# facebookresearch/holo_diffusion

Measured on AMD Instinct MI355X. Metric: denoise-steps/sec + rendered-rays/sec, 64^3x32 grid @400^2 render, higher is better.
Workload: dtype f32

## Files before the change

### holo_diffusion_amd/csrc/holo_kernels.h

```cpp
#pragma once
#include <stddef.h>
#include <stdint.h>

#include "conv_weights.h"
#include "holo_knobs.h"

struct HoloCtx {
  int device;
  int num_cus;
  int deterministic = 0;
};

namespace holo {

enum class ConvKernel : int32_t {
  Gather = 0,
  Halo = 1,
  RowTile = 2,
  Wino2 = 4,
  Bf16Wide = 5,
  Wino3 = 6,
  Stream1x1 = 7,
  Bf16Persistent = 8,
  S2Bf16 = 9,
// ... 11 lines not shown
  int OD, OH, OW;
  int stride, pad, ksz;
  int Cout;
  const float* w;
  int CoutP, CinP;
  const float* coef;
  int act;
  const float* bias;
  const float* residual;
  float* out;
  const float* skip_src0;
  const float* skip_src1;
  int skip_C0, skip_C1;
  const float* skip_w;
  const uint16_t* w_bf;
  const uint16_t* skip_w_bf;
  int bf16;
  int skip_CinP;
  const float* skip_bias;
  double* stats;
  float* partial;
  int nsplit;
  int chunks_per_split;
  int skip_chunks_per_split;
  int tz;
  int grid_x;
  int stagger_ticks;
  unsigned long long* dbg;
  ConvKernel kernel;
  const float* w_wino2;
  const float* skip_w_wino2;
  const float* w_wino3;
  const float* skip_w_wino3;
  const uint16_t* w_bft;
  const uint16_t* skip_w_bft;
  int in_bf16;
  int res_bf16;
  int out_bf16;
  uint16_t* qkv_q;
  uint16_t* qkv_k;
  uint16_t* qkv_vt;
  float qkv_scale;
  int qkv_T, qkv_CH, qkv_H;
  int qkv_sb, qkv_rows;
};

bool conv_s2_bf16_supported(const ConvParams& p);
int conv_s2_bf16_launch(const ConvParams& p, void* stream);

bool conv1x1_qkv_bf16_supported(const ConvParams& p);
void conv1x1_qkv_bf16_plan(ConvParams& p, int num_cus);
int conv1x1_qkv_bf16_launch(const ConvParams& p, void* stream);
bool conv1x1_bf16_stream_supported(const ConvParams& p);
void conv1x1_bf16_stream_plan(ConvParams& p, int num_cus);
int conv1x1_bf16_stream_slabs(const ConvParams& p);
int conv1x1_bf16_stream_launch(const ConvParams& p, void* stream);

int repack_conv_weight_wino3_launch(const float* w, float* out, int Cout, int Cin, int src_taps, int CoutP, int CinP,
                                    void* stream);
int conv_wino3_launch(const ConvParams& p, void* stream);
int conv_bf16p_launch(const ConvParams& p, void* stream);

size_t conv_plan(ConvParams& p, int num_cus, const Knobs& k, int plan_n = 0);
int conv_launch(const ConvParams& p, void* stream);
int conv_stats_slabs(const ConvParams& p);
double conv_flops(const ConvParams& p);
// ... 375 lines not shown
```

### holo_diffusion_amd/csrc/holo_knobs.h

```cpp
#pragma once

#include <stdint.h>
#include <stdlib.h>

namespace holo {

#ifdef HOLO_EMU
constexpr bool EMU_BUILD = true;
#else
constexpr bool EMU_BUILD = false;
#endif

constexpr int64_t KNOB_UNSET = INT64_MIN;

#define HOLO_KNOBS(X)                                                                                                      \
  X(num_cus, "HOLO_NUM_CUS", POS, 0, CTX, "planners size grids and split-K for this many CUs (default: the device's)")     \
  X(conv_wino, "HOLO_CONV_WINO", INT, 1, HANDLE, "0: no Winograd copies of the conv weights (forward and dgrad)")          \
  X(conv_wino3, "HOLO_CONV_WINO3", INT, 1, HANDLE_PLAN, "0: no F(2x2x2, 3x3x3) copies / conv_wino3_kernel never chosen")   \
  X(keep_intermediates, "HOLO_KEEP_INTERMEDIATES", CH, '1', HANDLE,                                                        \
    "1: the plan releases no activation, holo_unet_fetch_block works")                                                     \
  X(render_v1, "HOLO_RENDER_V1", SET, 0, HANDLE, "the ray-per-column render kernel for everything")                        \
  X(render2_nw, "HOLO_RENDER2_NW", INT, 0, HANDLE, "8: the 8-wave form of render2_kernel's 12-wave configurations")        \
  X(render2_nrm_nw, "HOLO_RENDER2_NRM_NW", INT, 0, HANDLE,                                                                 \
    "8: rendered normals two waves per SIMD instead of 10 waves (the emulation build always runs 8)")                      \
  X(render_wgs, "HOLO_RENDER_WGS", POS, 0, HANDLE, "persistent render workgroups (default: one per CU)")                   \
  X(render_xcd, "HOLO_RENDER_XCD", RAW, KNOB_UNSET, HANDLE,                                                                \
    "XCD ranges of the render tile order (default 8; 2 in the emulation build; <= 1: plain order)")                        \
  X(render_tail, "HOLO_RENDER_TAIL", RAW, KNOB_UNSET, HANDLE,                                                              \
    "4-ray tiles at the end of every XCD range handed out as single rays (default: about two rounds; 3 in the "            \
    "emulation build; 0: off)")                                                                                            \
  X(render_static_tiles, "HOLO_RENDER_STATIC_TILES", SET, 0, HANDLE, "static tile stride instead of the dynamic hand-out") \
  X(render_timeline, "HOLO_RENDER_TIMELINE", SET, 0, HANDLE, "per-phase clocks of every render launch (synchronises!)")    \
  X(mlp_mean_bwd_chunk, "HOLO_MLP_MEAN_BWD_CHUNK", POS, 0, HANDLE,                                                         \
    "voxels per chunk of holo_mlp_mean_backward (default: what fits 4 GiB of rows; the emulation build: always 2048)")     \
  X(conv_wino_small, "HOLO_CONV_WINO_SMALL", INT, 1, PLAN, "0: under-filled levels take 64-voxel tiles, not Winograd")     \
  X(conv_force_tz2, "HOLO_CONV_FORCE_TZ2", INT, 0, PLAN, "1: 128-voxel tiles (hence the Winograd kernels) on small grids") \
  X(conv_qkv_fused, "HOLO_CONV_QKV_FUSED", INT, 1, PLAN, "0: row-tile qkv convolution + attn_pack_kernel")                 \
  X(conv1x1_bf16_stream, "HOLO_CONV1X1_BF16_STREAM", INT, 1, PLAN, "0: the row-tile kernel for bf16 1x1x1 convolutions")   \
  X(conv1x1_stream_min_m, "HOLO_CONV1X1_STREAM_MIN_M", INT, 131072, PLAN,                                                  \
    "rows from which a raw-input fp32 1x1x1 convolution streams (0: never)")                                               \
  X(conv1x1_small, "HOLO_CONV1X1_SMALL", INT, 1, PLAN, "0: the row-tile kernel for the fp32 attention's 1x1x1 convs")      \
  X(conv_s2t, "HOLO_CONV_S2T", INT, -1, PLAN, "stride-2 bf16 halo kernel: 0 never, 1 wherever defined (default: by fill)") \
  X(conv_bf16t, "HOLO_CONV_BF16T", INT, -1, PLAN, "bf16 wide-tile kernel: 0 never, 1 everywhere (default: by fill / K)")   \
  X(conv_bf16p, "HOLO_CONV_BF16P", INT, -1, PLAN,                                                                          \
    "its persistent form: 0 never, 1 every wide-tile launch, 2 activated input too (default: raw input)")                  \
  X(conv_bf16p_wgs, "HOLO_CONV_BF16P_WGS", INT, 0, PLAN, "at most this many persistent workgroups (0: no cap)")            \
  X(conv_wino3_min_items, "HOLO_CONV_WINO3_MIN_ITEMS", INT, KNOB_UNSET, PLAN,                                              \
    "work items from which conv_wino3_kernel runs (default: num_cus / 2)")                                                 \
  X(no_skip_fusion, "HOLO_NO_SKIP_FUSION", SET, 0, PLAN, "a ResBlock's 1x1x1 skip always as its own launch")               \
  X(skip_fusion_below_r, "HOLO_SKIP_FUSION_BELOW_R", RAW, 64, PLAN,                                                        \
    "exact fp32: the skip is fused into the second convolution below this grid edge")                                      \
  X(no_flash_attn, "HOLO_NO_FLASH_ATTN", SET, 0, PLAN, "attention as GEMM + softmax + GEMM")                               \
  X(bf16_flash_min_t, "HOLO_BF16_FLASH_MIN_T", RAW, 1024, PLAN, "tokens from which the bf16 mode takes its bf16 attention") \
  X(flash_split, "HOLO_FLASH_SPLIT", INT, 0, PLAN, "key splits of the fp32 attention, clamped to [1, T/128] (0: by fill)") \
  X(flash_v2_ksplit, "HOLO_FLASH_V2_KSPLIT", INT, 0, PLAN,                                                                 \
    "key splits of the bf16 attention: 1..8 dividing T into multiples of 128, else ignored")                               \
  X(attn_exact, "HOLO_ATTN_EXACT", SET, 0, PLAN, "bf16 attention: the exact loop alone, no LAZY pass")                     \
  X(debug_timestep_load, "HOLO_DEBUG_TIMESTEP_LOAD", INT, 0, PLAN, "how time_embed_kernel loads the timesteps (see it)")   \
  X(dgrad_s2_direct, "HOLO_DGRAD_S2_DIRECT", CH, '1', PLAN, "1: conv_dgrad_s2_kernel for every Downsample dgrad")          \
  X(wgrad_tiles, "HOLO_WGRAD_TILES", POS, 0, PLAN, "> 0: the tile weight-gradient kernel instead of the row-staged one")   \
  X(wgrad_reduce_tile_min, "HOLO_WGRAD_REDUCE_TILE_MIN", RAW, 1024, PLAN,                                                  \
    "64-element tiles from which the weight-gradient reduce runs its tile form")                                           \
  X(debug_plan, "HOLO_DEBUG_PLAN", SET, 0, PLAN, "[plan] lines on stderr: what every convolution / attention launches")    \
  X(viewpool_bwd_v1, "HOLO_VIEWPOOL_BWD_V1", CH, '1', CALL, "1: the register-accumulating view-pool backward kernel")      \
  HOLO_KNOBS_DEV(X)

#ifdef HOLO_DEV_PROBES
#define HOLO_KNOBS_DEV(X)                                                                                                  \
  X(viewpool_bwd_probe, "HOLO_VIEWPOOL_BWD_PROBE", RAW, KNOB_UNSET, CALL,                                                  \
    "view-pool backward: 0 no pass 2, 2 pass 2 without its atomics, 10 + k the atomics of map k alone")                    \
  X(viewpool_bwd_occ, "HOLO_VIEWPOOL_BWD_OCC", CH, '3', CALL, "view-pool backward: 3 = the 166-register build")
#else
#define HOLO_KNOBS_DEV(X)
#endif

typedef int64_t knob_INT_t, knob_RAW_t, knob_POS_t;
typedef bool knob_SET_t, knob_CH_t;
static inline int64_t knob_INT(const char* e, int64_t dflt) { return e && e[0] ? strtoll(e, nullptr, 10) : dflt; }
static inline int64_t knob_RAW(const char* e, int64_t dflt) { return e ? atoll(e) : dflt; }
static inline bool knob_SET(const char* e, int) { return e != nullptr; }
static inline bool knob_CH(const char* e, char c) { return e && e[0] == c; }
// ... 17 lines not shown
```

### holo_diffusion_amd/csrc/kernels_conv.hip

```cpp
#include <stdio.h>
#include <stdlib.h>

#include "holo_common.h"
#include "holo_kernels.h"

namespace holo {

namespace {

constexpr int BM = 128;
constexpr int BK = 32;
constexpr int LDK = 36;

__device__ __forceinline__ float silu_f(float v) { return v / (1.0f + __expf(-v)); }
__device__ __forceinline__ float silu_fast(float v) { return v * holo_rcp(1.0f + __expf(-v)); }

__device__ __forceinline__ float bf16_load(const uint16_t* p) { return __uint_as_float((uint32_t)(*p) << 16); }
__device__ __forceinline__ uint16_t bf16_round(float v) { return (uint16_t)(pack_bf16x2(v, 0.f) & 0xffffu); }
__device__ __forceinline__ float4 ld_act4(const float* base, int64_t idx, int bf) {
  if (bf) {
    const uint2 u = *reinterpret_cast<const uint2*>(reinterpret_cast<const uint16_t*>(base) + idx);
    return make_float4(__uint_as_float(u.x << 16), __uint_as_float(u.x & 0xffff0000u), __uint_as_float(u.y << 16),
                       __uint_as_float(u.y & 0xffff0000u));
  }
// ... 2326 lines not shown
      const int64_t s2t = k.conv_s2t;
      if (s2t != 0 && conv_s2_bf16_supported(p) && ((Mc / 128) * (p.Cout / 64) >= num_cus / 4 || s2t == 1))
        return ConvKernel::S2Bf16;
      return p.Cout >= 64 ? ConvKernel::RowTile : ConvKernel::Gather;
    }
    const int64_t bt = k.conv_bf16t;
    if (p.bf16 == 1 && p.in_bf16 && p.w_bft && (!p.skip_w || p.skip_w_bft) && (p.OD % 8) == 0 && (p.OH % 8) == 0 &&
        (p.OW % 8) == 0 && (p.Cout % 32) == 0 && (p.C0 % 8) == 0 && (p.skip_C0 % 8) == 0 && ((p.skip_C0 + p.skip_C1) % 8) == 0 &&
        (p.Cout >= 64 || !p.skip_w) && bt != 0 &&
        (t8 >= target || Cin + (p.skip_w ? p.skip_C0 + p.skip_C1 : 0) >= BF16T_LONG_K || bt == 1)) {
      const int64_t bp = k.conv_bf16p;
      const int wgs = num_cus & ~7;
      if (bp != 0 && (bp == 1 || bp == 2 || !p.coef) &&
          ((bf16t_split(p, t8, ncc16, num_cus).n == 1 && wgs >= 8 && t8 >= wgs) || bp == 1) &&
          (p.C1 == 0 || (p.C0 % 16) == 0) &&
          (!p.skip_w || (((p.skip_C0 + p.skip_C1) % 32) == 0 && (p.skip_C1 == 0 || (p.skip_C0 % 32) == 0))) &&
          src_vox < ((int64_t)1 << 24))
        return ConvKernel::Bf16Persistent;
      return ConvKernel::Bf16Wide;
    }
    if (tz == 2 && k.conv_wino3 != 0 && p.w_wino3 && p.bf16 == 0 && !p.in_bf16 && !p.out_bf16 && p.Cout >= 64 &&
        (p.Cout % 64) == 0 && (!p.skip_w || p.skip_w_wino3) && (p.OH % 8) == 0 && (p.OW % 8) == 0 && (p.OD % 2) == 0 &&
        (!p.coef || p.act) &&
        (int64_t)p.N * src_vox * (cmax > skmax ? cmax : skmax) * 4 < ((int64_t)1 << 32) &&
        (int64_t)wino3_split(t3, ncc, num_cus).n * Mc * p.Cout * 4 < ((int64_t)1 << 32) &&
        (!p.stats || (Mc / 128) * p.Cout * 16 < ((int64_t)1 << 32)) &&
        (!p.skip_w || ((p.skip_C0 % 16) == 0 && (p.skip_C1 % 4) == 0)) &&
        t3 * wino3_split(t3, ncc, num_cus).n >= (k.conv_wino3_min_items != KNOB_UNSET ? k.conv_wino3_min_items : num_cus / 2))
      return ConvKernel::Wino3;
    if (tz == 2 && (wino2_wide || (p.w_wino2 && p.bf16 == 0 && p.Cout == 32 && !p.skip_w))) return ConvKernel::Wino2;
    return ConvKernel::Halo;
  }();
  p.kernel = kernel;

  switch (kernel) {
    case ConvKernel::Qkv:
    case ConvKernel::Bf16Stream1x1:
    case ConvKernel::Stream1x1:
    case ConvKernel::Small1x1:
      p.nsplit = 1;
      p.chunks_per_split = ncc;
      if (kernel == ConvKernel::Qkv) conv1x1_qkv_bf16_plan(p, num_cus);
      if (kernel == ConvKernel::Bf16Stream1x1) conv1x1_bf16_stream_plan(p, num_cus);
      break;
    case ConvKernel::S2Bf16:
      p.nsplit = 1;
      p.chunks_per_split = Cin / 16;
      break;
    case ConvKernel::RowTile: {
      const int64_t t2 = cdiv(Mc, SM_ROWS) * cdiv(p.Cout, 64);
      const int64_t tgt = SM_SPLIT_WGS_PER_CU * (int64_t)num_cus;
      const int nall = nchunks + nsk;
      const int max_split = nall / SG > 1 ? nall / SG : 1;
      const KSplit s = ksplit(t2 < tgt ? cdiv(tgt, t2) : 1, max_split, nall);
      p.nsplit = s.n;
      p.chunks_per_split = s.cps;
      break;
    }
    case ConvKernel::Gather: {
      const int max_split = nchunks / 4 > 1 ? nchunks / 4 : 1;
      const KSplit s = ksplit(tiles < target ? cdiv(target, tiles) : 1, max_split, nchunks);
      p.nsplit = s.n;
      p.chunks_per_split = s.cps;
      break;
    }
    case ConvKernel::Bf16Wide: {
// ... 54 lines not shown
    int B, vpb;
    gn_stats_geometry(p.Cout < 1024 ? p.Cout : 1024, V, &B, &vpb);
    return B;
  }
  switch (p.kernel) {
    case ConvKernel::Bf16Wide:
    case ConvKernel::Bf16Persistent:
      return (int)(V / 512);
    case ConvKernel::Halo:
      if (p.bf16 == 2 && p.w_bf && p.Cout >= 64 && !p.skip_w) return (int)(V / 32);
      [[fallthrough]];
    case ConvKernel::Wino2:
    case ConvKernel::Wino3:
      return (int)(V / (64 * p.tz)) * (p.Cout >= 64 ? 1 : 2);
    case ConvKernel::RowTile:
      return V % SM_ROWS == 0 ? (int)(V / SM_ROWS) : 0;
    case ConvKernel::S2Bf16:
      return (int)(V / 128);
    case ConvKernel::Bf16Stream1x1:
      return conv1x1_bf16_stream_slabs(p);
    case ConvKernel::Small1x1:
      return (int)(V / 16);
    default:
      return 0;
  }
}

double conv_flops(const ConvParams& p) {
  const double M = (double)p.N * p.OD * p.OH * p.OW;
  return 2.0 * M * p.Cout * ((double)(p.C0 + p.C1) * p.ksz * p.ksz * p.ksz + (p.skip_w ? p.skip_C0 + p.skip_C1 : 0));
}

double conv_exec_flops(const ConvParams& p) {
  const double taps = p.kernel == ConvKernel::Wino3 ? 8.0 : p.kernel == ConvKernel::Wino2 ? 12.0 : 0.0;
  if (taps == 0.0) return conv_flops(p);
  const double M = (double)p.N * p.OD * p.OH * p.OW;
  return 2.0 * M * p.Cout * ((double)(p.C0 + p.C1) * taps + (p.skip_w ? p.skip_C0 + p.skip_C1 : 0));
}

int conv_launch(const ConvParams& p, void* stream) {
  const int Cin = p.C0 + p.C1;
  if ((Cin & 3) || (p.C0 & 3) || (p.Cout & 3) || (p.src1 && (p.C0 % BK))) {
    set_error("conv_launch: unsupported channel counts C0=%d C1=%d Cout=%d", p.C0, p.C1, p.Cout);
    return -1;
  }
  if (p.nsplit > 1 && !p.partial) {
    set_error("conv_launch: split-K without scratch");
    return -1;
  }
  const int64_t M = (int64_t)p.N * p.OD * p.OH * p.OW;
  const bool wide = p.Cout >= 64;
  const bool sk = p.skip_w != nullptr;
  const int bn = wide ? 64 : 32;
  dim3 block(256);
  dim3 hgrid((unsigned)p.grid_x, (unsigned)cdiv(p.Cout, bn), (unsigned)p.nsplit);
  switch (p.kernel) {
    case ConvKernel::Gather: {
      dim3 grid((unsigned)cdiv(M, BM), (unsigned)cdiv(p.Cout, bn), (unsigned)p.nsplit);
      if (wide) {
        HOLO_LAUNCH(conv_igemm_kernel<2>, grid, block, stream, p);
      } else {
        HOLO_LAUNCH(conv_igemm_kernel<1>, grid, block, stream, p);
      }
      break;
    }
    case ConvKernel::Halo: {
      if (p.bf16 == 2 && p.w_bf && wide && !sk) {
// ... 157 lines not shown
```

### holo_diffusion_amd/csrc/kernels_conv3.hip

```cpp
#include <stdio.h>
#include <stdlib.h>

#include <type_traits>
#include <utility>

#include "holo_common.h"
#include "holo_kernels.h"

#ifndef W3_PROBE
#define W3_PROBE 0
#endif
#ifndef W3_WDIST
#define W3_WDIST 3
#endif
#ifndef W3_ENTRY
#define W3_ENTRY conv_wino3_launch
#endif

namespace holo {

namespace {

#ifdef HOLO_EMU
#define W3_KARGS(kp) const ConvParams* kp = &p
#else
#define W3_KARGS(kp)                                                                                        \
  auto kp = (const ConvParams __attribute__((address_space(4)))*)(__builtin_amdgcn_kernarg_segment_ptr()); \
  asm volatile("" : "+s"(kp))
#endif

constexpr int W3_BK = 32;
constexpr int W3_RS = 36;
constexpr int W3_HY = 10, W3_HX = 10;
constexpr int W3_PLANE = W3_HY * W3_HX;
constexpr int W3_HALO = 4 * W3_PLANE * W3_RS;
constexpr int W3_WSUB = 4 * 256;
constexpr int W3_WCHUNK = 32 * W3_WSUB;
constexpr int W3_WSKIP = 4 * W3_WSUB;

__device__ __forceinline__ float w3_silu(float v) { return v * holo_rcp(1.0f + __expf(-v)); }

struct w3q {
  f32x2 lo, hi;
};
__device__ __forceinline__ w3q w3_ld(const float* p) {
  const float4 v = *reinterpret_cast<const float4*>(p);
// ... 24 lines not shown
#else
typedef __amdgpu_buffer_rsrc_t w3_rsrc;
typedef unsigned w3u4 __attribute__((ext_vector_type(4)));
__device__ __forceinline__ w3_rsrc w3_make_rsrc(const void* p) {
  return __builtin_amdgcn_make_buffer_rsrc(const_cast<void*>(p), 0, 0xffffffff, 0x00020000);
}
__device__ __forceinline__ w3_rsrc w3_make_rsrc_n(const void* p, unsigned nbytes) {
  return __builtin_amdgcn_make_buffer_rsrc(const_cast<void*>(p), 0, nbytes, 0x00020000);
}
__device__ __forceinline__ w3q w3_bld(w3_rsrc r, unsigned voff, unsigned soff) {
  const w3u4 v = __builtin_amdgcn_raw_buffer_load_b128(r, voff, soff, 0);
  return w3q{f32x2{__uint_as_float(v.x), __uint_as_float(v.y)}, f32x2{__uint_as_float(v.z), __uint_as_float(v.w)}};
}
__device__ __forceinline__ float w3_bld1(w3_rsrc r, unsigned voff, unsigned soff) {
  return __uint_as_float(__builtin_amdgcn_raw_buffer_load_b32(r, voff, soff, 0));
}
__device__ __forceinline__ void w3_bst1(w3_rsrc r, unsigned voff, unsigned soff, float v) {
  __builtin_amdgcn_raw_buffer_store_b32(__float_as_uint(v), r, voff, soff, 0);
}
__device__ __forceinline__ void w3_bst_d2(w3_rsrc r, unsigned voff, unsigned soff, double a, double b) {
  const unsigned long long ua = __builtin_bit_cast(unsigned long long, a), ub = __builtin_bit_cast(unsigned long long, b);
  const w3u4 v = {(unsigned)ua, (unsigned)(ua >> 32), (unsigned)ub, (unsigned)(ub >> 32)};
  __builtin_amdgcn_raw_buffer_store_b128(v, r, voff, soff, 0);
}
#endif
__device__ __forceinline__ w3q w3_add(const w3q& a, const w3q& b) { return w3q{pk_add(a.lo, b.lo), pk_add(a.hi, b.hi)}; }
__device__ __forceinline__ w3q w3_sub(const w3q& a, const w3q& b) { return w3q{pk_sub(a.lo, b.lo), pk_sub(a.hi, b.hi)}; }

template <class F, int... K>
__device__ __forceinline__ void w3_static_for(F&& f, std::integer_sequence<int, K...>) {
  (f(std::integral_constant<int, K>{}), ...);
}

static_assert(std::is_trivially_copyable<ConvParams>::value && std::is_standard_layout<ConvParams>::value,
              "W3_KARGS reads ConvParams straight from the kernarg segment");
template <bool SKIP, bool XF>
__global__ __launch_bounds__(256, 1) void conv_wino3_kernel(ConvParams p) {
  __shared__ __attribute__((aligned(16))) float s_halo[2 * W3_HALO];

  const int tid = threadIdx.x;
  const int lane = tid & 63;
  const int wn = HOLO_UNIFORM(tid >> 6);
  const int lj = lane & 15;
  const int kq = lane >> 4;
  const int Cin = p.C0 + p.C1;
  const int ncc = (Cin + W3_BK - 1) / W3_BK;
  const int SCin = p.skip_C0 + p.skip_C1;
  const int ntx = p.OW >> 3, nty = p.OH >> 3, ntz = p.OD >> 1;
  const int ntiles = p.N * ntz * nty * ntx;
  const int ny = (p.Cout + 63) >> 6;
  const int nitems = ntiles * ny * p.nsplit;
  const int SD = p.ups ? (p.ID >> 1) : p.ID;
  const int SH = p.ups ? (p.IH >> 1) : p.IH;
  const int SW = p.ups ? (p.IW >> 1) : p.IW;
  const int wnsl = p.CoutP >> 4;
  const int64_t M = (int64_t)p.N * p.OD * p.OH * p.OW;

  struct Item {
    int n, tz0, ty0, tx0, n0, split, cc_begin, cc_end, sk_begin, sk_end;
  };
  const int X = ((W3_PROBE & 128) && (nty & 7) == 0 && (gridDim.x & 7) == 0) ? 8 : 1;
  const int ntyh = nty / X;
  const int lane_x = (int)blockIdx.x % X, G = (int)gridDim.x / X, nq = nitems / X;
  auto chunks_of = [&](Item& I) {
    I.cc_begin = I.split * p.chunks_per_split;
    I.cc_end = min(I.cc_begin + p.chunks_per_split, ncc);
    const int nsk = SKIP ? (SCin + W3_BK - 1) / W3_BK : 0;
    I.sk_begin = min(I.split * p.skip_chunks_per_split, nsk);
    I.sk_end = min(I.sk_begin + p.skip_chunks_per_split, nsk);
  };
// ... 64 lines not shown
#pragma unroll
    for (int i = 0; i < 4; ++i) {
      int y = I.ty0 - 1 + (int)((h_yx >> (8 * i)) & 15u), x = I.tx0 - 1 + (int)((h_yx >> (8 * i + 4)) & 15u);
      const unsigned ok = (unsigned)((unsigned)y < (unsigned)p.IH) & (unsigned)((unsigned)x < (unsigned)p.IW);
      y = min(max(y, 0), p.IH - 1) >> p.ups;
      x = min(max(x, 0), p.IW - 1) >> p.ups;
      h_cvalid |= ok << i;
      h_vox[i] = (unsigned)(y * SW + x);
    }
  };
  auto halo_chunk = [&](const Item& I, int cc) {
    int c = cc * W3_BK + q * 4;
    h_chvalid = c < Cin;
    if (!h_chvalid) c = 0;
    const bool second = p.src1 != nullptr && cc * W3_BK >= p.C0;
    const int Cs = second ? p.C1 : p.C0;
    const int cs = second ? c - p.C0 : c;
    if (XF) {
      const float4* cf = reinterpret_cast<const float4*>(p.coef + ((int64_t)I.n * Cin + c) * 2);
      h_c01 = cf[0], h_c23 = cf[1];
    }
    const unsigned cbytes = (unsigned)Cs * 4u;
    h_second = second;
#pragma unroll
    for (int pl = 0; pl < 4; ++pl) h_zoff[pl] = h_zvox[pl] * cbytes;
#pragma unroll
    for (int i = 0; i < 4; ++i) h_off[i] = h_vox[i] * cbytes + (unsigned)cs * 4u;
  };
  auto halo_setup = [&](const Item& I, int cc) {
    halo_tile(I);
    halo_chunk(I, cc);
  };
  auto halo_load = [&](int i, int pl) {
    const w3q v = h_second ? w3_bld(rsrc1, h_off[i], h_zoff[pl]) : w3_bld(rsrc0, h_off[i], h_zoff[pl]);
    if (i & 1)
      hrB[pl] = v;
    else
      hrA[pl] = v;
  };
  auto commit_item_on = [&](w3q(&H)[4], int i, float* buf) {
    f32x2* V[8] = {&H[0].lo, &H[0].hi, &H[1].lo, &H[1].hi, &H[2].lo, &H[2].hi, &H[3].lo, &H[3].hi};
    if (XF && !(W3_PROBE & 64)) {
      f32x2 e[8];
      const f32x2 ca[2] = {f32x2{h_c01.x, h_c01.z}, f32x2{h_c23.x, h_c23.z}}, cb[2] = {f32x2{h_c01.y, h_c01.w}, f32x2{h_c23.y, h_c23.w}};
#pragma unroll
      for (int j = 0; j < 8; ++j) *V[j] = pk_fma(*V[j], ca[j & 1], cb[j & 1]);
      __builtin_amdgcn_sched_barrier(0);
#pragma unroll
      for (int j = 0; j < 8; ++j) e[j] = pk_mul(*V[j], f32x2{-1.4426950408889634f, -1.4426950408889634f});
      __builtin_amdgcn_sched_barrier(0);
#pragma unroll
      for (int j = 0; j < 8; ++j) e[j] = f32x2{holo_exp2(e[j].x), holo_exp2(e[j].y)};
      __builtin_amdgcn_sched_barrier(0);
#pragma unroll
      for (int j = 0; j < 8; ++j) e[j] = pk_add(e[j], f32x2{1.f, 1.f});
      __builtin_amdgcn_sched_barrier(0);
#pragma unroll
      for (int j = 0; j < 8; ++j) e[j] = f32x2{holo_rcp(e[j].x), holo_rcp(e[j].y)};
      __builtin_amdgcn_sched_barrier(0);
#pragma unroll
      for (int j = 0; j < 8; ++j) *V[j] = pk_mul(*V[j], e[j]);
      __builtin_amdgcn_sched_barrier(0);
    }
    const float kc = (h_chvalid && ((h_cvalid >> i) & 1u)) ? 1.f : 0.f;
#pragma unroll
    for (int j = 0; j < 8; ++j) {
      const float keep = ((h_zvalid >> (j >> 1)) & 1u) ? kc : 0.f;
      *V[j] = pk_mul(*V[j], f32x2{keep, keep});
    }
    const int col = min((tid >> 3) + 32 * i, W3_PLANE - 1);
    float* dst = buf + col * W3_RS + q * 4;
    const w3q o0 = w3_sub(H[0], H[2]), o1 = w3_add(H[1], H[2]), o2 = w3_sub(H[2], H[1]), o3 = w3_sub(H[1], H[3]);
    *reinterpret_cast<float4*>(dst + 0 * W3_PLANE * W3_RS) = make_float4(o0.lo.x, o0.lo.y, o0.hi.x, o0.hi.y);
    *reinterpret_cast<float4*>(dst + 1 * W3_PLANE * W3_RS) = make_float4(o1.lo.x, o1.lo.y, o1.hi.x, o1.hi.y);
    *reinterpret_cast<float4*>(dst + 2 * W3_PLANE * W3_RS) = make_float4(o2.lo.x, o2.lo.y, o2.hi.x, o2.hi.y);
    *reinterpret_cast<float4*>(dst + 3 * W3_PLANE * W3_RS) = make_float4(o3.lo.x, o3.lo.y, o3.hi.x, o3.hi.y);
  };
  auto commit_item = [&](int i, float* buf) {
    if (i & 1)
      commit_item_on(hrB, i, buf);
    else
      commit_item_on(hrA, i, buf);
  };

  f32x4 acc[64];
  const int a_off = ((2 * (lj & 3)) * W3_HX + 2 * (lj >> 2)) * W3_RS + kq * 4;
  w3q P[4][4];
  w3q Y[2][4];
  auto load_patch_row = [&](const float* buf, int step, int a) {
    const float* base = buf + a_off + ((step >> 1) * W3_PLANE + a * W3_HX) * W3_RS + (step & 1) * 16;
#pragma unroll
    for (int b = 0; b < 4; ++b) P[a][b] = w3_ld(base + b * W3_RS);
  };
  auto xform_row_half = [&](int a, int h) {
    if (h == 0) {
      const w3q t0 = w3_sub(P[a][0], P[a][2]), t3 = w3_sub(P[a][1], P[a][3]);
      P[a][0] = t0, P[a][3] = t3;
    } else {
      const w3q t1 = w3_add(P[a][1], P[a][2]), t2 = w3_sub(P[a][2], P[a][1]);
      P[a][1] = t1, P[a][2] = t2;
    }
  };
  auto yform1 = [&](int xy, int b) {
    return xy == 0 ? w3_sub(P[0][b], P[2][b]) : xy == 1 ? w3_add(P[1][b], P[2][b]) : xy == 2 ? w3_sub(P[2][b], P[1][b]) : w3_sub(P[1][b], P[3][b]);
  };
  w3q Bdummy[4] = {};
  w3q Bw[4][4];
  auto mfma1 = [&](f32x4& c, const w3q& A, const w3q& B, int e, bool first, bool zero = false) {
#if W3_PROBE & 8
    HOLO_SINK8(A.lo.x, A.lo.y, A.hi.x, A.hi.y, B.lo.x, B.lo.y, B.hi.x, B.hi.y);
    return;
#endif
    const float a = e == 0 ? A.lo.x : e == 1 ? A.lo.y : e == 2 ? A.hi.x : A.hi.y;
    const float b = e == 0 ? B.lo.x : e == 1 ? B.lo.y : e == 2 ? B.hi.x : B.hi.y;
    if (zero) {
      if (first)
        HOLO_MFMA16_ZERO_FIRST(c, a, b);
      else
        HOLO_MFMA16_ZERO(c, a, b);
    } else if (first) {
      HOLO_MFMA16_ACC_FIRST(c, a, b);
    } else {
      HOLO_MFMA16_ACC(c, a, b);
    }
  };

  auto mfma16 = [&](f32x4& c0, f32x4& c1, f32x4& c2, f32x4& c3, const w3q (&A)[4], const w3q (&B)[4]) {
#pragma unroll
    for (int e = 0; e < 4; ++e) {
      mfma1(c0, A[0], B[0], e, e == 0);
      mfma1(c1, A[1], B[1], e, false);
      mfma1(c2, A[2], B[2], e, false);
      mfma1(c3, A[3], B[3], e, false);
    }
  };

  unsigned long long* dbg = p.dbg ? p.dbg + (int64_t)blockIdx.x * 8 : nullptr;
  if (dbg && tid == 0) dbg[0] = HOLO_PROBE_CLOCK();

  int it = (int)blockIdx.x / X;
  if (it >= nq) return;
  Item cur, nxt;
  decode(it, cur, lane_x);
  auto w_of = [&](const Item& I, int cc) { return (unsigned)((cc * wnsl + (I.n0 >> 4) + wn) * W3_WCHUNK) * 4u; };
  const w3_rsrc rsrcw = w3_make_rsrc(p.w_wino3);
  const unsigned lane16 = (unsigned)lane * 16u;
  auto w_ld = [&](unsigned ubase, int ofs_floats) { return w3_bld(rsrcw, lane16, ubase + (unsigned)ofs_floats * 4u); };

  int stage = 0;
  int cc = cur.cc_begin;
#pragma unroll
  for (int g = 0; g < W3_WDIST; ++g)
#pragma unroll
    for (int t = 0; t < 4; ++t) Bw[g][t] = w_ld(w_of(cur, cc), g * W3_WSUB + t * 256);
  halo_setup(cur, cc);
#pragma unroll
  for (int hp = 0; hp < 2; ++hp) {
#pragma unroll
    for (int i = 2 * hp; i < 2 * hp + 2; ++i)
#pragma unroll
      for (int pl = 0; pl < 4; ++pl) halo_load(i, pl);
#pragma unroll
    for (int i = 2 * hp; i < 2 * hp + 2; ++i) commit_item(i, s_halo);
  }
  __syncthreads();
#pragma unroll
  for (int a = 0; a < 4; ++a) load_patch_row(s_halo, 0, a);
#pragma unroll
  for (int a = 0; a < 4; ++a) {
    xform_row_half(a, 0);
    xform_row_half(a, 1);
  }
#pragma unroll
  for (int b = 0; b < 4; ++b) Y[0][b] = yform1(0, b);
  if (dbg && tid == 0) dbg[1] = HOLO_PROBE_CLOCK();

#ifdef W3_TIMELINE
  unsigned long long tl[7] = {0, 0, 0, 0, 0, 0, 0};
#endif
  for (;;) {
#if W3_PROBE & 8
#pragma unroll
    for (int s = 0; s < 64; ++s)
#pragma unroll
      for (int r = 0; r < 4; ++r) acc[s][r] = 0.f;
#endif
    cc = cur.cc_begin;
    auto stage_body = [&](auto opens_c) __attribute__((always_inline)) {
      constexpr bool opens = decltype(opens_c)::value;
      const bool last_chunk = cc + 1 == cur.cc_end;
      const bool go = last_chunk && it + G < nq;
      Item adv;
      advance(cur, adv);
      nxt.n = go ? adv.n : cur.n, nxt.tz0 = go ? adv.tz0 : cur.tz0, nxt.ty0 = go ? adv.ty0 : cur.ty0;
      nxt.tx0 = go ? adv.tx0 : cur.tx0, nxt.n0 = go ? adv.n0 : cur.n0, nxt.split = go ? adv.split : cur.split;
      nxt.cc_begin = go ? adv.cc_begin : cur.cc_begin, nxt.cc_end = go ? adv.cc_end : cur.cc_end;
      nxt.sk_begin = go ? adv.sk_begin : cur.sk_begin, nxt.sk_end = go ? adv.sk_end : cur.sk_end;
      const int ncc_ = go ? adv.cc_begin : last_chunk ? cc : cc + 1;
      const float* buf = s_halo + (stage & 1) * W3_HALO;
      float* obuf = s_halo + ((stage + 1) & 1) * W3_HALO;
      const unsigned wp = w_of(cur, cc), wnext = w_of(nxt, ncc_);
#ifdef W3_TIMELINE
      const unsigned long long t_stage = HOLO_PROBE_CLOCK();
#endif
      auto group = [&](auto gc) {
        constexpr int g = decltype(gc)::value, st = g >> 2, xy = g & 3;
#ifdef W3_TIMELINE
        const unsigned long long tA0 = clock64();
#endif
        if (g == 28) __syncthreads();
#ifdef W3_TIMELINE
        const unsigned long long tA = clock64();
        if (g == 28) tl[5] += tA - tA0;
#endif
        auto slot = [&](auto kc) {
          constexpr int k = decltype(kc)::value;
          mfma1(acc[(st >> 1) * 16 + xy * 4 + (k & 3)], Y[g & 1][k & 3], Bw[g & 3][k & 3], k >> 2, k == 0,
                opens && (st & 1) == 0 && (k >> 2) == 0);
          if ((k & 3) == 0 && !(W3_PROBE & 2)) {
            const unsigned wsrc = g + W3_WDIST < 32 ? wp : wnext;
            constexpr int wofs = (g + W3_WDIST < 32 ? g + W3_WDIST : g + W3_WDIST - 32) * W3_WSUB + (k >> 2) * 256;
            if (W3_PROBE & 16)
              Bdummy[k >> 2] = w_ld(wsrc, wofs);
            else
              Bw[(g + W3_WDIST) & 3][k >> 2] = w_ld(wsrc, wofs);
          }
          if (xy == 3 && k < 8 && !(W3_PROBE & 4)) {
            const float* pb = st < 7 ? buf : obuf;
            constexpr int nstep = st < 7 ? st + 1 : 0;
            const float* base = pb + a_off + ((nstep >> 1) * W3_PLANE + (k >> 1) * W3_HX) * W3_RS + (nstep & 1) * 16;
            P[k >> 1][(2 * k) & 3] = w3_ld(base + ((2 * k) & 3) * W3_RS);
            P[k >> 1][(2 * k + 1) & 3] = w3_ld(base + ((2 * k + 1) & 3) * W3_RS);
          }
          if (((g >= 1 && g <= 4) || (g >= 16 && g <= 19)) && (k == 2 || k == 10) && !(W3_PROBE & 1)) {
            constexpr int hl = (g >= 16 ? g - 16 : g >= 1 ? g - 1 : 0) * 2 + (k == 10 ? 1 : 0);
            halo_load((g >= 16 ? 2 : 0) + (hl >> 2), hl & 3);
          }
          __builtin_amdgcn_sched_barrier(0);
        };
        w3_static_for(slot, std::make_integer_sequence<int, 16>{});
#ifdef W3_TIMELINE
        const unsigned long long tB = clock64();
        tl[0] += tB - tA;
#endif
        if (!(W3_PROBE & 4)) {
          if (xy == 3) {
#pragma unroll
            for (int a = 0; a < 4; ++a) {
              xform_row_half(a, 0);
              xform_row_half(a, 1);
            }
          }
#pragma unroll
          for (int b = 0; b < 4; ++b) Y[(g + 1) & 1][b] = yform1((xy + 1) & 3, b);
        }
        if (!(W3_PROBE & 1)) {
          if (g == 0) halo_setup(nxt, ncc_);
          if (!(W3_PROBE & 32)) {
            if (g == 8) commit_item(0, obuf);
            if (g == 12) commit_item(1, obuf);
            if (g == 20) commit_item(2, obuf);
            if (g == 24) commit_item(3, obuf);
          }
        }
        __builtin_amdgcn_sched_barrier(0);
#ifdef W3_TIMELINE
        tl[g == 0 ? 4 : (g == 8 || g == 12 || g == 20 || g == 24) ? 3 : xy == 3 ? 2 : 1] += clock64() - tB;
        if (g == 0) tl[6] += 1;
#endif
      };
      w3_static_for(group, std::make_integer_sequence<int, 32>{});
#ifdef W3_TIMELINE
      if (dbg && tid == 0) dbg[6] += HOLO_PROBE_CLOCK() - t_stage;
#endif
      ++stage;
    };
    stage_body(std::true_type{});
    int cc_end = cur.cc_end;
    HOLO_LAUNDER_S(cc_end);
    while (++cc < cc_end) stage_body(std::false_type{});
    W3_KARGS(kp);
    if (SKIP) {
      const int nsg = (cur.sk_end - cur.sk_begin) * 4;
      if (nsg > 0) {
        const w3_rsrc rs0 = w3_make_rsrc(kp->skip_src0), rs1 = w3_make_rsrc(kp->skip_src1 ? kp->skip_src1 : kp->skip_src0);
        const w3_rsrc rsw = w3_make_rsrc(kp->skip_w_wino3);
        const int yt = lj & 3, xt = lj >> 2;
        unsigned vrel[4];
#pragma unroll
        for (int d = 0; d < 4; ++d) vrel[d] = (unsigned)((2 * yt + (d >> 1)) * kp->OW + 2 * xt + (d & 1));
        const unsigned vtile = (unsigned)(((cur.n * kp->OD + cur.tz0) * kp->OH + cur.ty0) * kp->OW + cur.tx0);
        const unsigned zvox = (unsigned)(kp->OH * kp->OW);
        const unsigned wbase = (unsigned)((cur.n0 >> 4) + wn) * (unsigned)W3_WSKIP * 4u;
        auto skip_load = [&](int sg, int slot) {
          const int sc = cur.sk_begin + (sg >> 2), half = (sg >> 1) & 1, dz = sg & 1;
          const int c0 = sc * W3_BK + half * 16;
          const bool pad = c0 >= SCin;
          const bool second = !pad && c0 >= kp->skip_C0;
          const unsigned Cs = (unsigned)(second ? kp->skip_C1 : kp->skip_C0);
          const unsigned cs = pad ? 0u : (unsigned)(second ? c0 - kp->skip_C0 : c0);
          const unsigned soff = ((vtile + (unsigned)dz * zvox) * Cs + cs) * 4u;
          const unsigned wsoff = (unsigned)sc * (unsigned)wnsl * (unsigned)W3_WSKIP * 4u + wbase + (unsigned)((half * 2 + dz) * 4) * 1024u;
          const unsigned koff = (unsigned)min(kq * 4, max((int)Cs - (int)cs - 4, 0)) * 4u;
#pragma unroll
// ... 47 lines not shown
      if (direct && kp->bias) bv = w3_bld1(w3_make_rsrc(kp->bias), e_lj, cbase * 4u);
      if (direct && kp->skip_bias) bv += w3_bld1(w3_make_rsrc(kp->skip_bias), e_lj, cbase * 4u);
      const unsigned vtile = (unsigned)(((cur.n * kp->OD + cur.tz0) * kp->OH + cur.ty0) * kp->OW + cur.tx0);
      const unsigned sbase = vtile * cout4 + cbase * 4u;
      const unsigned obase = direct ? sbase : sbase + (unsigned)cur.split * ((unsigned)M * cout4);
      const unsigned zstride = (unsigned)(kp->OH * kp->OW) * cout4, ystride = (unsigned)kp->OW * cout4;
      const w3_rsrc rs_out = w3_make_rsrc(direct ? kp->out : kp->partial);
      const w3_rsrc rs_res = w3_make_rsrc_n(kp->residual, HOLO_UNIFORM(has_res ? 0xffffffffu : 0u));
      auto vofs = [&](int r, int dz, int dy, int dx) {
        return (unsigned)dz * zstride + (unsigned)(2 * r + dy) * ystride + (unsigned)dx * cout4;
      };
      float res[2][2][2][2];
      auto load_res = [&](int r) {
#pragma unroll
        for (int dz = 0; dz < 2; ++dz)
#pragma unroll
          for (int dy = 0; dy < 2; ++dy)
#pragma unroll
            for (int dx = 0; dx < 2; ++dx) res[r & 1][dz][dy][dx] = w3_bld1(rs_res, e_voff, sbase + vofs(r, dz, dy, dx));
      };
      load_res(0);
      float ssum = 0.f, ssq = 0.f;
#pragma unroll
      for (int r = 0; r < 4; ++r) {
        if (r < 3) load_res(r + 1);
        f32x2 oz[2][2][2];
#pragma unroll
        for (int zp = 0; zp < 2; ++zp) {
          f32x2 oy[4][2];
#pragma unroll
          for (int xy = 0; xy < 4; ++xy) {
            const int s0 = (2 * zp) * 16 + xy * 4, s1 = s0 + 16;
            float a0, a1, a2, a3, b0, b1, b2, b3;
            HOLO_ACC_READ(a0, acc[s0 + 0], r);
            HOLO_ACC_READ(b0, acc[s1 + 0], r);
            HOLO_ACC_READ(a1, acc[s0 + 1], r);
            HOLO_ACC_READ(b1, acc[s1 + 1], r);
            HOLO_ACC_READ(a2, acc[s0 + 2], r);
            HOLO_ACC_READ(b2, acc[s1 + 2], r);
            HOLO_ACC_READ(a3, acc[s0 + 3], r);
            HOLO_ACC_READ(b3, acc[s1 + 3], r);
            const f32x2 m0 = f32x2{a0, b0}, m1 = f32x2{a1, b1}, m2 = f32x2{a2, b2}, m3 = f32x2{a3, b3};
            oy[xy][0] = pk_add(pk_add(m0, m1), m2);
            oy[xy][1] = pk_sub(pk_sub(m1, m2), m3);
          }
#pragma unroll
          for (int dx = 0; dx < 2; ++dx) {
            oz[zp][0][dx] = pk_add(pk_add(oy[0][dx], oy[1][dx]), oy[2][dx]);
            oz[zp][1][dx] = pk_sub(pk_sub(oy[1][dx], oy[2][dx]), oy[3][dx]);
          }
          __builtin_amdgcn_sched_barrier(0);
        }
        if (SKIP && r == 3 && cur.sk_end > cur.sk_begin) {
          const float* nbuf = s_halo + (stage & 1) * W3_HALO;
#pragma unroll
          for (int a4 = 0; a4 < 4; ++a4) load_patch_row(nbuf, 0, a4);
        }
#pragma unroll
        for (int dy = 0; dy < 2; ++dy)
#pragma unroll
          for (int dx = 0; dx < 2; ++dx) {
            const f32x2 za = oz[0][dy][dx], zb = oz[1][dy][dx];
            float o0 = (za.x + za.y) + zb.x;
            float o1 = (za.y - zb.x) - zb.y;
            if (direct) {
              o0 = (o0 + res[r & 1][0][dy][dx]) + bv;
              o1 = (o1 + res[r & 1][1][dy][dx]) + bv;
              ssum += o0 + o1;
              ssq = fmaf(o0, o0, fmaf(o1, o1, ssq));
            }
            w3_bst1(rs_out, e_voff, obase + vofs(r, 0, dy, dx), o0);
            w3_bst1(rs_out, e_voff, obase + vofs(r, 1, dy, dx), o1);
          }
        __builtin_amdgcn_sched_barrier(0);
// ... 9 lines not shown
          const int slab = ((cur.tz0 >> 1) * nty + (cur.ty0 >> 3)) * ntx + (cur.tx0 >> 3);
          const unsigned rec = ((unsigned)(cur.n * tiles_per_sample + slab) * (unsigned)kp->Cout + cbase) * 16u;
          w3_bst_d2(w3_make_rsrc(kp->stats), e_lj * 4u, rec, (double)s1, (double)s2);
        }
      }
    }
    if (dbg && tid == 0) {
      const unsigned long long t_now = HOLO_PROBE_CLOCK();
      atomicAdd(dbg + 5, t_now - dbg[2]);
      dbg[3] = t_now;
      atomicAdd(dbg + 7, 1ull);
    }
    it += G;
    if (it >= nq) break;
    if (SKIP && cur.sk_end > cur.sk_begin) {
#pragma unroll
      for (int a4 = 0; a4 < 4; ++a4) {
        xform_row_half(a4, 0);
        xform_row_half(a4, 1);
      }
#pragma unroll
      for (int b4 = 0; b4 < 4; ++b4) Y[0][b4] = yform1(0, b4);
    }
    cur = nxt;
  }
#ifdef W3_TIMELINE
  if (p.dbg && tid == 0) {
    unsigned long long* d = p.dbg + ((int64_t)gridDim.x + blockIdx.x) * 8;
#pragma unroll
    for (int i = 0; i < 7; ++i) d[i] = tl[i];
  }
#endif
}

__global__ __launch_bounds__(256) void repack_conv_weight_wino3_kernel(const float* __restrict__ w, float* __restrict__ out,
                                                                       int Cout, int Cin, int src_taps, int CoutP, int CinP) {
  const int per = src_taps == 27 ? W3_WCHUNK : W3_WSKIP;
  const int nsl = CoutP >> 4;
  const int64_t total = (int64_t)(CinP >> 5) * nsl * per;
  const double G[4][3] = {{1.0, 0.0, 0.0}, {0.5, 0.5, 0.5}, {0.5, -0.5, 0.5}, {0.0, 0.0, 1.0}};
  for (int64_t i = (int64_t)blockIdx.x * blockDim.x + threadIdx.x; i < total; i += (int64_t)gridDim.x * blockDim.x) {
    const int e = (int)(i & 3);
    const int lj = (int)((i >> 2) & 15);
    const int kq = (int)((i >> 6) & 3);
    int g = (int)((i % per) >> 8);
    const int64_t blk = i / per;
    const int slice = (int)(blk % nsl);
    const int cc = (int)(blk / nsl);
    const int co = slice * 16 + lj;
    float v = 0.f;
    if (src_taps == 27) {
      const int xx = g & 3, xy = (g >> 2) & 3, half = (g >> 4) & 1, xz = g >> 5;
      const int ci = cc * 32 + half * 16 + kq * 4 + e;
      if (ci < Cin && co < Cout) {
        const float* src = w + ((int64_t)co * Cin + ci) * 27;
        double u = 0.0;
        for (int kz = 0; kz < 3; ++kz)
          for (int ky = 0; ky < 3; ++ky)
            for (int kx = 0; kx < 3; ++kx) u += G[xz][kz] * G[xy][ky] * G[xx][kx] * (double)holo_ld_sys(src + kz * 9 + ky * 3 + kx);
        v = (float)u;
      }
    } else {
      const int d = g & 3, dz = (g >> 2) & 1, half = g >> 3;
      const int ci = cc * 32 + half * 16 + kq * 4 + e;
      if (ci < Cin && co < Cout) {
        const float s = ((dz + (d >> 1) + (d & 1)) & 1) ? -1.f : 1.f;
// ... 7 lines not shown
}

#if W3_PROBE == 0 && !defined(W3_TIMELINE)
int64_t conv_wino3_weight_floats(int CoutP, int CinP, int src_taps) {
  return (int64_t)(CinP >> 5) * (CoutP >> 4) * (src_taps == 27 ? W3_WCHUNK : W3_WSKIP);
}

int repack_conv_weight_wino3_launch(const float* w, float* out, int Cout, int Cin, int src_taps, int CoutP, int CinP,
                                    void* stream) {
  const int64_t total = conv_wino3_weight_floats(CoutP, CinP, src_taps);
  int64_t blocks = (total + 255) / 256;
  if (blocks > 8192) blocks = 8192;
  HOLO_LAUNCH(repack_conv_weight_wino3_kernel, dim3((unsigned)blocks), dim3(256), stream, w, out, Cout, Cin, src_taps, CoutP,
              CinP);
  return 0;
}

#endif

int W3_ENTRY(const ConvParams& p, void* stream) {
  if (!p.w_wino3 || (p.skip_w && !p.skip_w_wino3) || (p.OD & 1) || (p.OH & 7) || (p.OW & 7) || (p.Cout & 63) ||
      (p.coef && !p.act)) {
    set_error("conv_wino3_launch: unsupported shape / weights not prepared");
    return -1;
  }
  const int ncc = (p.C0 + p.C1 + W3_BK - 1) / W3_BK;
  const int64_t out_bytes = (int64_t)p.N * p.OD * p.OH * p.OW * p.Cout * 4;
  if (p.nsplit < 1 || p.chunks_per_split < 1 || (int64_t)(p.nsplit - 1) * p.chunks_per_split >= ncc ||
      out_bytes * p.nsplit >= ((int64_t)1 << 32)) {
    set_error("conv_wino3_launch: empty K split, or output beyond 32-bit byte offsets");
    return -1;
  }
  const dim3 grid((unsigned)p.grid_x), block(256);
  if (p.skip_w && p.coef) {
    HOLO_LAUNCH((conv_wino3_kernel<true, true>), grid, block, stream, p);
  } else if (p.skip_w) {
    HOLO_LAUNCH((conv_wino3_kernel<true, false>), grid, block, stream, p);
  } else if (p.coef) {
    HOLO_LAUNCH((conv_wino3_kernel<false, true>), grid, block, stream, p);
  } else {
    HOLO_LAUNCH((conv_wino3_kernel<false, false>), grid, block, stream, p);
  }
  return 0;
}

}
```

Baseline: 165.6.

## Add 27-tap Winograd F(2,3) form for nearest-upsampled input convolutions

Adds an upsampling specialisation of the Winograd 3x3x3 kernel. With a x2 nearest-upsampled input, one of the four transformed taps per axis is redundant, so it runs 3 live taps per axis (27 instead of 64 pseudo-taps). That skips dead MFMA groups, weight loads, halo transform outputs and accumulator reads. This adds a new kernel instantiation and relies on the duplicated-input identity holding exactly. It is enabled by default for upsample convs without a fused skip or coefficients.

After: 169.2, median of 6. 2.2% higher.

```diff
diff --git a/holo_diffusion_amd/csrc/holo_kernels.h b/holo_diffusion_amd/csrc/holo_kernels.h
--- a/holo_diffusion_amd/csrc/holo_kernels.h
+++ b/holo_diffusion_amd/csrc/holo_kernels.h
@@ -67,6 +67,7 @@
   const float* skip_w_wino2;
   const float* w_wino3;
   const float* skip_w_wino3;
+  int wino3_up;
   const uint16_t* w_bft;
   const uint16_t* skip_w_bft;
   int in_bf16;
diff --git a/holo_diffusion_amd/csrc/holo_knobs.h b/holo_diffusion_amd/csrc/holo_knobs.h
--- a/holo_diffusion_amd/csrc/holo_knobs.h
+++ b/holo_diffusion_amd/csrc/holo_knobs.h
@@ -47,6 +47,8 @@
   X(conv_bf16p_wgs, "HOLO_CONV_BF16P_WGS", INT, 0, PLAN, "at most this many persistent workgroups (0: no cap)")            \
   X(conv_wino3_min_items, "HOLO_CONV_WINO3_MIN_ITEMS", INT, KNOB_UNSET, PLAN,                                              \
     "work items from which conv_wino3_kernel runs (default: num_cus / 2)")                                                 \
+  X(conv_wino3_up, "HOLO_CONV_WINO3_UP", INT, 1, PLAN,                                                                     \
+    "0: upsampling convolutions on conv_wino3_kernel's generic form (64 pseudo-taps), not its 27-tap form")               \
   X(no_skip_fusion, "HOLO_NO_SKIP_FUSION", SET, 0, PLAN, "a ResBlock's 1x1x1 skip always as its own launch")               \
   X(skip_fusion_below_r, "HOLO_SKIP_FUSION_BELOW_R", RAW, 64, PLAN,                                                        \
     "exact fp32: the skip is fused into the second convolution below this grid edge")                                      \
diff --git a/holo_diffusion_amd/csrc/kernels_conv.hip b/holo_diffusion_amd/csrc/kernels_conv.hip
--- a/holo_diffusion_amd/csrc/kernels_conv.hip
+++ b/holo_diffusion_amd/csrc/kernels_conv.hip
@@ -2382,6 +2382,7 @@
     return ConvKernel::Halo;
   }();
   p.kernel = kernel;
+  p.wino3_up = kernel == ConvKernel::Wino3 && p.ups && !p.coef && !p.skip_w && k.conv_wino3_up != 0 ? 1 : 0;
 
   switch (kernel) {
     case ConvKernel::Qkv:
@@ -2502,7 +2503,8 @@
 }
 
 double conv_exec_flops(const ConvParams& p) {
-  const double taps = p.kernel == ConvKernel::Wino3 ? 8.0 : p.kernel == ConvKernel::Wino2 ? 12.0 : 0.0;
+  const double wino3_taps = p.wino3_up ? 27.0 / 8.0 : 8.0;
+  const double taps = p.kernel == ConvKernel::Wino3 ? wino3_taps : p.kernel == ConvKernel::Wino2 ? 12.0 : 0.0;
   if (taps == 0.0) return conv_flops(p);
   const double M = (double)p.N * p.OD * p.OH * p.OW;
   return 2.0 * M * p.Cout * ((double)(p.C0 + p.C1) * taps + (p.skip_w ? p.skip_C0 + p.skip_C1 : 0));
diff --git a/holo_diffusion_amd/csrc/kernels_conv3.hip b/holo_diffusion_amd/csrc/kernels_conv3.hip
--- a/holo_diffusion_amd/csrc/kernels_conv3.hip
+++ b/holo_diffusion_amd/csrc/kernels_conv3.hip
@@ -12,6 +12,9 @@
 #endif
 #ifndef W3_WDIST
 #define W3_WDIST 3
+#endif
+#ifndef W3_UP_ONE_REQ
+#define W3_UP_ONE_REQ 0
 #endif
 #ifndef W3_ENTRY
 #define W3_ENTRY conv_wino3_launch
@@ -102,10 +105,26 @@
   (f(std::integral_constant<int, K>{}), ...);
 }
 
+template <bool UP>
+constexpr int w3_live(int i) {
+  return UP && i == 2 ? 3 : i;
+}
+constexpr bool w3_dead_set(int s) { return (s >> 4) == 2 || ((s >> 2) & 3) == 2 || (s & 3) == 2; }
+template <bool UP>
+constexpr int w3_wofs(int gi, int ti) {
+  constexpr int NL = UP ? 3 : 4;
+  const int st = gi / NL;
+  return ((((w3_live<UP>(st >> 1) * 2 + (st & 1)) * 4 + w3_live<UP>(gi % NL)) * 4) + w3_live<UP>(ti)) * 256;
+}
+
 static_assert(std::is_trivially_copyable<ConvParams>::value && std::is_standard_layout<ConvParams>::value,
               "W3_KARGS reads ConvParams straight from the kernarg segment");
-template <bool SKIP, bool XF>
-__global__ __launch_bounds__(256, 1) void conv_wino3_kernel(ConvParams p) {
+template <bool SKIP, bool XF, bool UP>
+__device__ __forceinline__ void conv_wino3_body(const ConvParams& p) {
+  static_assert(!UP || (!SKIP && !XF), "the upsampling form: raw input, no fused skip");
+  constexpr int NL = UP ? 3 : 4, NG = 2 * NL * NL, NK = 4 * NL, NR = UP ? 6 : 4;
+  constexpr int GH0 = 1, GH1 = UP ? 7 : 16, GC0 = UP ? 6 : 8, GC1 = UP ? 8 : 12, GC2 = UP ? 12 : 20, GC3 = UP ? 14 : 24;
+  constexpr int GBAR = UP ? 16 : 28;
   __shared__ __attribute__((aligned(16))) float s_halo[2 * W3_HALO];
 
   const int tid = threadIdx.x;
@@ -236,6 +255,7 @@
     halo_chunk(I, cc);
   };
   auto halo_load = [&](int i, int pl) {
+    if (UP && W3_UP_ONE_REQ && pl == 2) return;
     const w3q v = h_second ? w3_bld(rsrc1, h_off[i], h_zoff[pl]) : w3_bld(rsrc0, h_off[i], h_zoff[pl]);
     if (i & 1)
       hrB[pl] = v;
@@ -243,6 +263,7 @@
       hrA[pl] = v;
   };
   auto commit_item_on = [&](w3q(&H)[4], int i, float* buf) {
+    if (UP && W3_UP_ONE_REQ) H[2] = H[1];
     f32x2* V[8] = {&H[0].lo, &H[0].hi, &H[1].lo, &H[1].hi, &H[2].lo, &H[2].hi, &H[3].lo, &H[3].hi};
     if (XF && !(W3_PROBE & 64)) {
       f32x2 e[8];
@@ -274,10 +295,13 @@
     }
     const int col = min((tid >> 3) + 32 * i, W3_PLANE - 1);
     float* dst = buf + col * W3_RS + q * 4;
-    const w3q o0 = w3_sub(H[0], H[2]), o1 = w3_add(H[1], H[2]), o2 = w3_sub(H[2], H[1]), o3 = w3_sub(H[1], H[3]);
+    const w3q o0 = w3_sub(H[0], H[2]), o1 = w3_add(H[1], H[2]), o3 = w3_sub(H[1], H[3]);
     *reinterpret_cast<float4*>(dst + 0 * W3_PLANE * W3_RS) = make_float4(o0.lo.x, o0.lo.y, o0.hi.x, o0.hi.y);
     *reinterpret_cast<float4*>(dst + 1 * W3_PLANE * W3_RS) = make_float4(o1.lo.x, o1.lo.y, o1.hi.x, o1.hi.y);
-    *reinterpret_cast<float4*>(dst + 2 * W3_PLANE * W3_RS) = make_float4(o2.lo.x, o2.lo.y, o2.hi.x, o2.hi.y);
+    if (!UP) {
+      const w3q o2 = w3_sub(H[2], H[1]);
+      *reinterpret_cast<float4*>(dst + 2 * W3_PLANE * W3_RS) = make_float4(o2.lo.x, o2.lo.y, o2.hi.x, o2.hi.y);
+    }
     *reinterpret_cast<float4*>(dst + 3 * W3_PLANE * W3_RS) = make_float4(o3.lo.x, o3.lo.y, o3.hi.x, o3.hi.y);
   };
   auto commit_item = [&](int i, float* buf) {
@@ -300,6 +324,8 @@
     if (h == 0) {
       const w3q t0 = w3_sub(P[a][0], P[a][2]), t3 = w3_sub(P[a][1], P[a][3]);
       P[a][0] = t0, P[a][3] = t3;
+    } else if (UP) {
+      P[a][1] = w3_add(P[a][1], P[a][2]);
     } else {
       const w3q t1 = w3_add(P[a][1], P[a][2]), t2 = w3_sub(P[a][2], P[a][1]);
       P[a][1] = t1, P[a][2] = t2;
@@ -309,7 +335,7 @@
     return xy == 0 ? w3_sub(P[0][b], P[2][b]) : xy == 1 ? w3_add(P[1][b], P[2][b]) : xy == 2 ? w3_sub(P[2][b], P[1][b]) : w3_sub(P[1][b], P[3][b]);
   };
   w3q Bdummy[4] = {};
-  w3q Bw[4][4];
+  w3q Bw[NR][4];
   auto mfma1 = [&](f32x4& c, const w3q& A, const w3q& B, int e, bool first, bool zero = false) {
 #if W3_PROBE & 8
     HOLO_SINK8(A.lo.x, A.lo.y, A.hi.x, A.hi.y, B.lo.x, B.lo.y, B.hi.x, B.hi.y);
@@ -329,6 +355,12 @@
     }
   };
 
+  auto acc_read = [&](int s, int r) {
+    float v = 0.f;
+    if (!(UP && w3_dead_set(s))) HOLO_ACC_READ(v, acc[s], r);
+    return v;
+  };
+
   auto mfma16 = [&](f32x4& c0, f32x4& c1, f32x4& c2, f32x4& c3, const w3q (&A)[4], const w3q (&B)[4]) {
 #pragma unroll
     for (int e = 0; e < 4; ++e) {
@@ -356,7 +388,7 @@
 #pragma unroll
   for (int g = 0; g < W3_WDIST; ++g)
 #pragma unroll
-    for (int t = 0; t < 4; ++t) Bw[g][t] = w_ld(w_of(cur, cc), g * W3_WSUB + t * 256);
+    for (int t = 0; t < NL; ++t) Bw[g][w3_live<UP>(t)] = w_ld(w_of(cur, cc), w3_wofs<UP>(g, t));
   halo_setup(cur, cc);
 #pragma unroll
   for (int hp = 0; hp < 2; ++hp) {
@@ -376,7 +408,8 @@
     xform_row_half(a, 1);
   }
 #pragma unroll
-  for (int b = 0; b < 4; ++b) Y[0][b] = yform1(0, b);
+  for (int b = 0; b < 4; ++b)
+    if (!UP || b != 2) Y[0][b] = yform1(0, b);
   if (dbg && tid == 0) dbg[1] = HOLO_PROBE_CLOCK();
 
 #ifdef W3_TIMELINE
@@ -408,47 +441,48 @@
       const unsigned long long t_stage = HOLO_PROBE_CLOCK();
 #endif
       auto group = [&](auto gc) {
-        constexpr int g = decltype(gc)::value, st = g >> 2, xy = g & 3;
+        constexpr int g = decltype(gc)::value, sti = g / NL, xyi = g % NL;
+        constexpr int xz = w3_live<UP>(sti >> 1), half = sti & 1, xy = w3_live<UP>(xyi);
 #ifdef W3_TIMELINE
         const unsigned long long tA0 = clock64();
 #endif
-        if (g == 28) __syncthreads();
+        if (g == GBAR) __syncthreads();
 #ifdef W3_TIMELINE
         const unsigned long long tA = clock64();
-        if (g == 28) tl[5] += tA - tA0;
+        if (g == GBAR) tl[5] += tA - tA0;
 #endif
         auto slot = [&](auto kc) {
-          constexpr int k = decltype(kc)::value;
-          mfma1(acc[(st >> 1) * 16 + xy * 4 + (k & 3)], Y[g & 1][k & 3], Bw[g & 3][k & 3], k >> 2, k == 0,
-                opens && (st & 1) == 0 && (k >> 2) == 0);
-          if ((k & 3) == 0 && !(W3_PROBE & 2)) {
-            const unsigned wsrc = g + W3_WDIST < 32 ? wp : wnext;
-            constexpr int wofs = (g + W3_WDIST < 32 ? g + W3_WDIST : g + W3_WDIST - 32) * W3_WSUB + (k >> 2) * 256;
+          constexpr int k = decltype(kc)::value, xx = w3_live<UP>(k % NL), e = k / NL;
+          mfma1(acc[xz * 16 + xy * 4 + xx], Y[g & 1][xx], Bw[g % NR][xx], e, k == 0, opens && half == 0 && e == 0);
+          if ((k & 3) == 0 && (k >> 2) < NL && !(W3_PROBE & 2)) {
+            constexpr int gn = g + W3_WDIST;
+            const unsigned wsrc = gn < NG ? wp : wnext;
+            constexpr int wofs = w3_wofs<UP>(gn < NG ? gn : gn - NG, k >> 2);
             if (W3_PROBE & 16)
               Bdummy[k >> 2] = w_ld(wsrc, wofs);
             else
-              Bw[(g + W3_WDIST) & 3][k >> 2] = w_ld(wsrc, wofs);
-          }
-          if (xy == 3 && k < 8 && !(W3_PROBE & 4)) {
-            const float* pb = st < 7 ? buf : obuf;
-            constexpr int nstep = st < 7 ? st + 1 : 0;
-            const float* base = pb + a_off + ((nstep >> 1) * W3_PLANE + (k >> 1) * W3_HX) * W3_RS + (nstep & 1) * 16;
+              Bw[gn % NR][w3_live<UP>(k >> 2)] = w_ld(wsrc, wofs);
+          }
+          if (xyi == NL - 1 && k < 8 && !(W3_PROBE & 4)) {
+            const float* pb = sti + 1 < 2 * NL ? buf : obuf;
+            constexpr int nsti = sti + 1 < 2 * NL ? sti + 1 : 0;
+            const float* base = pb + a_off + (w3_live<UP>(nsti >> 1) * W3_PLANE + (k >> 1) * W3_HX) * W3_RS + (nsti & 1) * 16;
             P[k >> 1][(2 * k) & 3] = w3_ld(base + ((2 * k) & 3) * W3_RS);
             P[k >> 1][(2 * k + 1) & 3] = w3_ld(base + ((2 * k + 1) & 3) * W3_RS);
           }
-          if (((g >= 1 && g <= 4) || (g >= 16 && g <= 19)) && (k == 2 || k == 10) && !(W3_PROBE & 1)) {
-            constexpr int hl = (g >= 16 ? g - 16 : g >= 1 ? g - 1 : 0) * 2 + (k == 10 ? 1 : 0);
-            halo_load((g >= 16 ? 2 : 0) + (hl >> 2), hl & 3);
+          if (((g >= GH0 && g < GH0 + 4) || (g >= GH1 && g < GH1 + 4)) && (k == 2 || k == 10) && !(W3_PROBE & 1)) {
+            constexpr int hl = (g >= GH1 ? g - GH1 : g >= GH0 ? g - GH0 : 0) * 2 + (k == 10 ? 1 : 0);
+            halo_load((g >= GH1 ? 2 : 0) + (hl >> 2), hl & 3);
           }
           __builtin_amdgcn_sched_barrier(0);
         };
-        w3_static_for(slot, std::make_integer_sequence<int, 16>{});
+        w3_static_for(slot, std::make_integer_sequence<int, NK>{});
 #ifdef W3_TIMELINE
         const unsigned long long tB = clock64();
         tl[0] += tB - tA;
 #endif
         if (!(W3_PROBE & 4)) {
-          if (xy == 3) {
+          if (xyi == NL - 1) {
 #pragma unroll
             for (int a = 0; a < 4; ++a) {
               xform_row_half(a, 0);
@@ -456,24 +490,25 @@
             }
           }
 #pragma unroll
-          for (int b = 0; b < 4; ++b) Y[(g + 1) & 1][b] = yform1((xy + 1) & 3, b);
+          for (int b = 0; b < 4; ++b)
+            if (!UP || b != 2) Y[(g + 1) & 1][b] = yform1(w3_live<UP>((xyi + 1) % NL), b);
         }
         if (!(W3_PROBE & 1)) {
           if (g == 0) halo_setup(nxt, ncc_);
           if (!(W3_PROBE & 32)) {
-            if (g == 8) commit_item(0, obuf);
-            if (g == 12) commit_item(1, obuf);
-            if (g == 20) commit_item(2, obuf);
-            if (g == 24) commit_item(3, obuf);
+            if (g == GC0) commit_item(0, obuf);
+            if (g == GC1) commit_item(1, obuf);
+            if (g == GC2) commit_item(2, obuf);
+            if (g == GC3) commit_item(3, obuf);
           }
         }
         __builtin_amdgcn_sched_barrier(0);
 #ifdef W3_TIMELINE
-        tl[g == 0 ? 4 : (g == 8 || g == 12 || g == 20 || g == 24) ? 3 : xy == 3 ? 2 : 1] += clock64() - tB;
+        tl[g == 0 ? 4 : (g == GC0 || g == GC1 || g == GC2 || g == GC3) ? 3 : xyi == NL - 1 ? 2 : 1] += clock64() - tB;
         if (g == 0) tl[6] += 1;
 #endif
       };
-      w3_static_for(group, std::make_integer_sequence<int, 32>{});
+      w3_static_for(group, std::make_integer_sequence<int, NG>{});
 #ifdef W3_TIMELINE
       if (dbg && tid == 0) dbg[6] += HOLO_PROBE_CLOCK() - t_stage;
 #endif
@@ -587,14 +622,10 @@
           for (int xy = 0; xy < 4; ++xy) {
             const int s0 = (2 * zp) * 16 + xy * 4, s1 = s0 + 16;
             float a0, a1, a2, a3, b0, b1, b2, b3;
-            HOLO_ACC_READ(a0, acc[s0 + 0], r);
-            HOLO_ACC_READ(b0, acc[s1 + 0], r);
-            HOLO_ACC_READ(a1, acc[s0 + 1], r);
-            HOLO_ACC_READ(b1, acc[s1 + 1], r);
-            HOLO_ACC_READ(a2, acc[s0 + 2], r);
-            HOLO_ACC_READ(b2, acc[s1 + 2], r);
-            HOLO_ACC_READ(a3, acc[s0 + 3], r);
-            HOLO_ACC_READ(b3, acc[s1 + 3], r);
+            a0 = acc_read(s0 + 0, r), b0 = acc_read(s1 + 0, r);
+            a1 = acc_read(s0 + 1, r), b1 = acc_read(s1 + 1, r);
+            a2 = acc_read(s0 + 2, r), b2 = acc_read(s1 + 2, r);
+            a3 = acc_read(s0 + 3, r), b3 = acc_read(s1 + 3, r);
             const f32x2 m0 = f32x2{a0, b0}, m1 = f32x2{a1, b1}, m2 = f32x2{a2, b2}, m3 = f32x2{a3, b3};
             oy[xy][0] = pk_add(pk_add(m0, m1), m2);
             oy[xy][1] = pk_sub(pk_sub(m1, m2), m3);
@@ -670,6 +701,12 @@
   }
 #endif
 }
+
+template <bool SKIP, bool XF>
+__global__ __launch_bounds__(256, 1) void conv_wino3_kernel(ConvParams p) {
+  conv_wino3_body<SKIP, XF, false>(p);
+}
+__global__ __launch_bounds__(256, 1) void conv_wino3_up_kernel(ConvParams p) { conv_wino3_body<false, false, true>(p); }
 
 __global__ __launch_bounds__(256) void repack_conv_weight_wino3_kernel(const float* __restrict__ w, float* __restrict__ out,
                                                                        int Cout, int Cin, int src_taps, int CoutP, int CinP) {
@@ -743,7 +780,13 @@
     return -1;
   }
   const dim3 grid((unsigned)p.grid_x), block(256);
-  if (p.skip_w && p.coef) {
+  if (p.wino3_up) {
+    if (!p.ups || p.coef || p.skip_w) {
+      set_error("conv_wino3_launch: the upsampling form takes raw x2 input without a fused skip");
+      return -1;
+    }
+    HOLO_LAUNCH(conv_wino3_up_kernel, grid, block, stream, p);
+  } else if (p.skip_w && p.coef) {
     HOLO_LAUNCH((conv_wino3_kernel<true, true>), grid, block, stream, p);
   } else if (p.skip_w) {
     HOLO_LAUNCH((conv_wino3_kernel<true, false>), grid, block, stream, p);
```
